# auniquesun/PPT

Measured on AMD Instinct MI355X. Metric: point-clouds/sec fwd+bwd, PointBERT 1024-pt ModelNet40, higher is better.
Workload: dtype f16; 1 GPU; C2: ModelNet40 1024-pt PointBERT (ULIP_PointBERT head_type=0, frozen backbone + PromptLearner), train-mode BN + DropPath, fwd + CE(ls 0.2) + bwd + AdamW; feed=resident, per_gpu_batch=32, global_batch=32, npoints=1024, classes=40, parallelism=dp1

## Files before the change

### include/ppt_hip.h

```cpp
#ifndef PPT_HIP_H
#define PPT_HIP_H

#include <stddef.h>
#include <stdint.h>

#ifdef __cplusplus
extern "C" {
#endif

#define PPT_OK 0
#define PPT_EINVAL (-1)
#define PPT_ELAUNCH (-2)
#define PPT_EUNSUPPORTED (-3)

#define PPT_F32 0
#define PPT_BF16 1
#define PPT_F16 2

const char *ppt_strerror(int code);
int ppt_abi_version(void);

int ppt_fps_f32(const float *xyz, int B, int N, int M, const int64_t *start, int64_t *out_idx,
                float *out_xyz, void *stream);

// ... 210 lines not shown
int ppt_attention_prefix_fwd(const void *qkv, void *out, float *lse, int C, int T, int P, int H, int hd, float scale, int dtype,
                             void *stream);
int ppt_attention_prefix_bwd(const void *qkv, const void *out, const void *dout, const float *lse, float *delta, void *dqkv,
                             float *workspace, int C, int T, int P, int H, int hd, float scale, int dtype, void *stream);

int ppt_conv1_stats(const float *pts, int64_t M, const float *w1, const float *b1, int C,
                    float *part_sum, float *part_sqsum, int *n_partials, void *stream);
int ppt_bn_finalize(const float *part_sum, const float *part_sqsum, int n_partials,
                    int rows_per_partial, int64_t count, int C, const float *gamma, const float *beta, float eps, int train,
                    float momentum, float *running_mean, float *running_var,
                    int64_t *num_batches_tracked, float *scale, float *shift, void *stream);
size_t ppt_bn_finalize_workspace_bytes(int n_partials, int C);
int ppt_bn_finalize_ws(const float *part_sum, const float *part_sqsum, int n_partials,
                       int rows_per_partial, int64_t count, int C, const float *gamma, const float *beta, float eps, int train,
                       float momentum, float *running_mean, float *running_var,
                       int64_t *num_batches_tracked, float *scale, float *shift,
                       float *mean_out , float *rstd_out ,
                       void *workspace, size_t workspace_bytes, void *stream);

int ppt_rows_stats_rows_per_partial(void);
int ppt_rows_stats_f32(const float *x, int64_t M, int C, float *part_sum, float *part_m2, void *stream);
int ppt_bn_rows_bwd_reduce(const float *dy, const float *x, const float *scale, const float *shift, const float *mean,
                           const float *rstd, int relu, int64_t M, int C, float *part_g, float *part_gx, void *stream);
int ppt_bn_rows_bwd_apply(const float *dy, const float *x, const float *scale, const float *shift, const float *mean,
                          const float *rstd, const float *sum_g, const float *sum_gx, int relu, int batch_stats, int64_t M,
                          int C, float *dx, void *dx_half, int half_dtype, void *stream);
int ppt_conv1_stats_max_partials(int64_t M);
int ppt_conv1_stats_rows_per_partial(void);

int ppt_gn_stats_chunks(int R);
int ppt_gn_bwd_chunks(int Q);
int ppt_gn_finish(const double *part, int B, int nch, int G, double n, double eps, int mode, float *out0, float *out1, void *stream);
int ppt_gn_stats(const float *y, int B, int R, int C, int G, double *part, void *stream);
int ppt_gn_lrelu_max(const float *y, const float *mean, const float *rstd, const float *gamma, const float *beta, int B, int Q, int K,
                     int C, int G, float slope, float *out, int32_t *arg, void *stream);
int ppt_gn_bwd_sums(const float *y, const float *dout, const float *out, const int32_t *arg, const float *mean, const float *rstd,
                    const float *gamma, int B, int Q, int K, int C, int G, float slope, double *psum, float *pgb, void *stream);
int ppt_gn_bwd_apply(const float *y, const float *dout, const float *out, const int32_t *arg, const float *mean, const float *rstd,
                     const float *gamma, const float *s12n, int B, int Q, int K, int C, int G, float slope, float *dy, void *stream);

int ppt_mini_pointnet_conv12_bf16(const float *pts, int64_t M, const float *w1, const float *b1, const float *a_scale,
                                  const float *a_shift, int C1, const void *W2, const float *bias2, int N, void *y2, void *gmax,
                                  void *stream);

int ppt_mini_pointnet_conv3_bf16(const void *A, int64_t M, int K, const void *W, const float *gterm, int N, void *y, float *part_sum,
                                 float *part_m2, void *stream);

int ppt_mini_pointnet_conv4_bf16(const void *A, int64_t M, int K, const float *a_scale, const float *a_shift, const void *W,
                                 const float *bias, int N, void *tok, void *stream);

int ppt_mini_pointnet_conv12_half(const float *pts, int64_t M, const float *w1, const float *b1, const float *a_scale,
                                  const float *a_shift, int C1, const void *W2, const float *bias2, int N, void *y2, void *gmax,
                                  int dtype, void *stream);
int ppt_mpn34_retile(const void *W4, void *W4_tiled, void *stream);
int ppt_mini_pointnet_conv34_half(const void *y2, int64_t M, const void *W3s, const float *gs, const void *W4_tiled,
                                  const float *bias4, void *tok, int dtype, void *stream);
int ppt_mini_pointnet_conv3_half(const void *A, int64_t M, int K, const void *W, const float *gterm, int N, void *y, float *part_sum,
                                 float *part_m2, int dtype, void *stream);
int ppt_mini_pointnet_conv4_half(const void *A, int64_t M, int K, const float *a_scale, const float *a_shift, const void *W,
                                 const float *bias, int N, void *tok, int dtype, void *stream);

int ppt_conv12_stats_bf16(const float *pts, int64_t M, const float *w1, const float *b1, const float *a_scale, const float *a_shift,
                          int C1, const void *W2, const float *bias2, int N, void *y2, float *part_sum, float *part_m2, void *stream);

int ppt_affine_conv_pool_bf16(const void *A, int64_t lda, int64_t M, int K, const float *a_scale, const float *a_shift, const void *W,
                              const float *bias, int N, int pool_rows, float *pmax, float *pmin, float *part_sum, float *part_m2,
                              void *stream);

int ppt_group_anchor_stats(const void *x, int x_dtype, const int64_t *idx, const int64_t *anchor, int B, int Nsrc, int S, int K,
                           int D, float *out, void *stream);
int ppt_pointmlp_cloud_rstd(const float *stats, int B, int S, double n, float *r, void *stream);
int ppt_pointmlp_pq(const float *PQ, const float *r, const int64_t *cidx, const float *c0, float *P, float *Q, int B, int N, int S,
                    int C, void *stream);
int ppt_bn_res_act_rows(const void *x, int x_dtype, const void *res, int res_dtype, int64_t M, int C, int pool, const float *scale,
                        const float *shift, const float *res_scale, const float *res_shift, void *y, int y_dtype, void *stream);

int ppt_gemm_tn_bf16(const void *A, int64_t lda, const void *B, int64_t ldb, int64_t M, int N1, int N2, int n_slices, float *part,
                     void *stream);
int ppt_gemm_tn_half(const void *A, int64_t lda, const void *B, int64_t ldb, int64_t M, int N1, int N2, int n_slices, float *part,
                     int dtype, void *stream);

int ppt_cross_entropy_rows(const float *logits, const int64_t *labels, float smoothing, int64_t R, int C, int64_t ignore_index,
                           float *loss, float *dlogits, float *partial, void *stream);

int ppt_rows_matmul_f32(const float *A, const float *W, int M, int K, int N, float alpha, float *out, void *stream);

int ppt_head_logits(const float *feat, const float *w, const float *text, const float *logit_scale, int B, int F, int E, int C,
                    float *spc, float *logits, void *stream);
int ppt_head_ce_bwd(const float *logits, const int64_t *labels, const float *spc, const float *text, float smoothing, int B,
                    int E, int C, float *loss, float *d_text, void *stream);

int ppt_linear3_gelu(const float *pts, int64_t M, const float *w, const float *b, int C, void *y,
                     int y_dtype, void *stream);
int ppt_cls_max_pool(const void *x, int x_dtype, int B, int T, int D, float *out, int32_t *argmax,
                     void *stream);
int ppt_three_nn_interp_fwd(const float *points1, int D1, const float *points2, int D2, const int64_t *idx, const float *dist,
                            int B, int N, int S, void *out, int out_dtype, int ld_out, float *weight_out, void *stream);
int ppt_scatter_rows_bwd(const int64_t *idx, const float *weight, const float *d_rows, int64_t ld, int col_off, int B, int E,
                         int rows_div, int S, int C, float *d_src, void *stream);
int ppt_sum_groups(const float *x, int64_t G, int k, int C, float *out, void *stream);

int ppt_gather_add(const void *P, int p_dtype, const float *Q, const int64_t *idx, int B, int Nsrc, int S, int K,
                   int C, void *y, int y_dtype, float *part_sum, float *part_m2, void *stream);
int ppt_pool_finish(const void *pmax, const void *pmin, int p_dtype, int G, int fold, int C, const float *scale,
                    const float *shift, void *out, int out_dtype, int64_t ld_out, void *stream);
int ppt_bn_act_rows(const float *x, int M, int C, const float *scale, const float *shift, const float *mask,
// ... 72 lines not shown
```

### ppt_amd/_lib.py

```python
import ctypes
import os

_HERE = os.path.dirname(os.path.abspath(__file__))
LIB_PATH = os.environ.get("PPT_HIP_LIB") or os.path.join(_HERE, "csrc", "libppt_hip.so")
_lib = None

PPT_F32, PPT_BF16, PPT_F16 = 0, 1, 2
A_PLAIN, A_AFFINE_RELU, A_CONV1 = 0, 1, 2
ACT_NONE, ACT_RELU, ACT_GELU, ACT_QUICKGELU = 0, 1, 2, 3

c_void_p, c_int, c_int64, c_float, c_size_t = (ctypes.c_void_p, ctypes.c_int, ctypes.c_int64,
                                               ctypes.c_float, ctypes.c_size_t)


class GemmParams(ctypes.Structure):
    _fields_ = [
        ("A", c_void_p), ("lda", c_int64), ("B", c_void_p), ("ldb", c_int64),
        ("C", c_void_p), ("ldc", c_int64), ("M", c_int), ("N", c_int), ("K", c_int),
        ("dtype", c_int), ("c_dtype", c_int),
        ("a_mode", c_int), ("a_scale", c_void_p), ("a_shift", c_void_p), ("pts", c_void_p),
        ("w1", c_void_p), ("b1", c_void_p),
        ("bias", c_void_p), ("group_add", c_void_p), ("group_rows", c_int), ("act", c_int),
        ("dact_pre", c_void_p), ("ld_dact", c_int64),
        ("row_scale", c_void_p), ("row_scale_rows", c_int),
# ... 118 lines not shown
                                  c_void_p, c_int, c_void_p, c_void_p, c_int, c_int, c_int, c_void_p]),
    "ppt_layernorm_fwd_sum": (c_int, [c_void_p, c_void_p, c_void_p, c_int, c_void_p, c_void_p, c_void_p, c_void_p, c_int,
                                      c_void_p, c_void_p, c_int, c_int, c_float, c_void_p]),
    "ppt_layernorm_bwd_sum": (c_int, [c_void_p, c_int, c_void_p, c_void_p, c_void_p, c_void_p, c_void_p, c_int,
                                      c_void_p, c_int, c_int, c_int, c_void_p]),
    "ppt_col_sums": (c_int, [c_void_p, c_int, c_int, c_int, c_int64, c_void_p, c_void_p]),
    "ppt_attention_fwd": (c_int, [c_void_p, c_void_p, c_void_p, c_int, c_int, c_int, c_int, c_float, c_int,
                                  c_int, c_void_p]),
    "ppt_attention_bwd": (c_int, [c_void_p, c_void_p, c_void_p, c_void_p, c_void_p, c_void_p, c_int, c_int,
                                  c_int, c_int, c_float, c_int, c_int, c_void_p]),
    "ppt_attention_prefix_workspace_bytes": (ctypes.c_size_t, [c_int, c_int, c_int, c_int]),
    "ppt_pointmlp_cloud_rstd": (c_int, [c_void_p, c_int, c_int, ctypes.c_double, c_void_p, c_void_p]),
    "ppt_pointmlp_pq": (c_int, [c_void_p, c_void_p, c_void_p, c_void_p, c_void_p, c_void_p, c_int, c_int, c_int, c_int, c_void_p]),
    "ppt_attention_bwd_split16": (c_int, [c_void_p, c_void_p, c_void_p, c_void_p, c_void_p, c_void_p, c_void_p, c_int, c_int, c_int, c_int, c_int, c_float, c_int, c_void_p]),
    "ppt_attention_fwd_split16": (c_int, [c_void_p, c_void_p, c_void_p, c_int, c_int, c_int, c_int, c_int, c_float, c_int, c_void_p]),
    "ppt_attention_prefix_fwd": (c_int, [c_void_p, c_void_p, c_void_p, c_int, c_int, c_int, c_int, c_int, c_float, c_int, c_void_p]),
    "ppt_attention_prefix_bwd": (c_int, [c_void_p, c_void_p, c_void_p, c_void_p, c_void_p, c_void_p, c_void_p, c_int, c_int, c_int,
                                         c_int, c_int, c_float, c_int, c_void_p]),
    "ppt_conv1_stats": (c_int, [c_void_p, c_int64, c_void_p, c_void_p, c_int, c_void_p, c_void_p,
                                ctypes.POINTER(c_int), c_void_p]),
    "ppt_conv1_stats_max_partials": (c_int, [c_int64]),
    "ppt_conv1_stats_rows_per_partial": (c_int, []),
    "ppt_bn_finalize": (c_int, [c_void_p, c_void_p, c_int, c_int, c_int64, c_int, c_void_p, c_void_p, c_float, c_int,
                                c_float, c_void_p, c_void_p, c_void_p, c_void_p, c_void_p, c_void_p]),
    "ppt_bn_finalize_ws": (c_int, [c_void_p, c_void_p, c_int, c_int, c_int64, c_int, c_void_p, c_void_p, c_float, c_int,
                                   c_float, c_void_p, c_void_p, c_void_p, c_void_p, c_void_p, c_void_p, c_void_p, c_void_p,
                                   ctypes.c_size_t, c_void_p]),
    "ppt_rows_stats_rows_per_partial": (c_int, []),
    "ppt_rows_stats_f32": (c_int, [c_void_p, c_int64, c_int, c_void_p, c_void_p, c_void_p]),
    "ppt_bn_rows_bwd_reduce": (c_int, [c_void_p, c_void_p, c_void_p, c_void_p, c_void_p, c_void_p, c_int, c_int64, c_int,
                                       c_void_p, c_void_p, c_void_p]),
    "ppt_bn_rows_bwd_apply": (c_int, [c_void_p, c_void_p, c_void_p, c_void_p, c_void_p, c_void_p, c_void_p, c_void_p, c_int,
                                      c_int, c_int64, c_int, c_void_p, c_void_p, c_int, c_void_p]),
    "ppt_bn_finalize_workspace_bytes": (ctypes.c_size_t, [c_int, c_int]),
    "ppt_gn_stats_chunks": (c_int, [c_int]),
    "ppt_gn_bwd_chunks": (c_int, [c_int]),
    "ppt_gn_stats": (c_int, [c_void_p, c_int, c_int, c_int, c_int, c_void_p, c_void_p]),
    "ppt_gn_lrelu_max": (c_int, [c_void_p, c_void_p, c_void_p, c_void_p, c_void_p, c_int, c_int, c_int, c_int, c_int, c_float,
                                 c_void_p, c_void_p, c_void_p]),
    "ppt_gn_bwd_sums": (c_int, [c_void_p, c_void_p, c_void_p, c_void_p, c_void_p, c_void_p, c_void_p, c_int, c_int, c_int, c_int,
                                c_int, c_float, c_void_p, c_void_p, c_void_p]),
    "ppt_gn_bwd_apply": (c_int, [c_void_p, c_void_p, c_void_p, c_void_p, c_void_p, c_void_p, c_void_p, c_void_p, c_int, c_int,
                                 c_int, c_int, c_int, c_float, c_void_p, c_void_p]),
    "ppt_mini_pointnet_conv12_bf16": (c_int, [c_void_p, c_int64, c_void_p, c_void_p, c_void_p, c_void_p, c_int, c_void_p, c_void_p,
                                              c_int, c_void_p, c_void_p, c_void_p]),
    "ppt_mini_pointnet_conv3_bf16": (c_int, [c_void_p, c_int64, c_int, c_void_p, c_void_p, c_int, c_void_p, c_void_p, c_void_p,
                                             c_void_p]),
    "ppt_mini_pointnet_conv4_bf16": (c_int, [c_void_p, c_int64, c_int, c_void_p, c_void_p, c_void_p, c_void_p, c_int, c_void_p,
                                             c_void_p]),
    "ppt_mini_pointnet_conv12_half": (c_int, [c_void_p, c_int64, c_void_p, c_void_p, c_void_p, c_void_p, c_int, c_void_p, c_void_p,
                                              c_int, c_void_p, c_void_p, c_int, c_void_p]),
    "ppt_mini_pointnet_conv3_half": (c_int, [c_void_p, c_int64, c_int, c_void_p, c_void_p, c_int, c_void_p, c_void_p, c_void_p,
                                             c_int, c_void_p]),
    "ppt_mpn34_retile": (c_int, [c_void_p, c_void_p, c_void_p]),
    "ppt_mini_pointnet_conv34_half": (c_int, [c_void_p, c_int64, c_void_p, c_void_p, c_void_p, c_void_p, c_void_p, c_int, c_void_p]),
    "ppt_mini_pointnet_conv4_half": (c_int, [c_void_p, c_int64, c_int, c_void_p, c_void_p, c_void_p, c_void_p, c_int, c_void_p,
                                             c_int, c_void_p]),
    "ppt_conv12_stats_bf16": (c_int, [c_void_p, c_int64, c_void_p, c_void_p, c_void_p, c_void_p, c_int, c_void_p, c_void_p,
                                      c_int, c_void_p, c_void_p, c_void_p, c_void_p]),
    "ppt_affine_conv_pool_bf16": (c_int, [c_void_p, c_int64, c_int64, c_int, c_void_p, c_void_p, c_void_p, c_void_p, c_int, c_int,
                                          c_void_p, c_void_p, c_void_p, c_void_p, c_void_p]),
    "ppt_group_anchor_stats": (c_int, [c_void_p, c_int, c_void_p, c_void_p, c_int, c_int, c_int, c_int, c_int, c_void_p, c_void_p]),
    "ppt_bn_res_act_rows": (c_int, [c_void_p, c_int, c_void_p, c_int, c_int64, c_int, c_int, c_void_p, c_void_p, c_void_p, c_void_p,
                                    c_void_p, c_int, c_void_p]),
    "ppt_gemm_tn_bf16": (c_int, [c_void_p, c_int64, c_void_p, c_int64, c_int64, c_int, c_int, c_int, c_void_p, c_void_p]),
    "ppt_gemm_tn_half": (c_int, [c_void_p, c_int64, c_void_p, c_int64, c_int64, c_int, c_int, c_int, c_void_p, c_int, c_void_p]),
    "ppt_head_logits": (c_int, [c_void_p, c_void_p, c_void_p, c_void_p, c_int, c_int, c_int, c_int, c_void_p, c_void_p, c_void_p]),
    "ppt_head_ce_bwd": (c_int, [c_void_p, c_void_p, c_void_p, c_void_p, c_float, c_int, c_int, c_int, c_void_p, c_void_p,
                                c_void_p]),
    "ppt_linear3_gelu": (c_int, [c_void_p, c_int64, c_void_p, c_void_p, c_int, c_void_p, c_int, c_void_p]),
    "ppt_cls_max_pool": (c_int, [c_void_p, c_int, c_int, c_int, c_int, c_void_p, c_void_p, c_void_p]),
    "ppt_adamw_step": (c_int, [c_void_p, c_void_p, c_void_p, c_void_p, c_int64, c_float, c_float, c_float, c_float, c_float, c_int,
                               c_float, c_void_p, c_void_p]),
    "ppt_adamw_multi": (c_int, [c_void_p, c_int, c_float, c_float, c_float, c_float, c_float, c_float, c_void_p, c_void_p]),
    "ppt_prompt_rows": (c_int, [c_void_p, c_void_p, c_void_p, c_void_p, c_int, c_int, c_void_p, c_void_p]),
    "ppt_prompt_rows_bwd": (c_int, [c_void_p, c_void_p, c_int, c_int, c_int, c_float, c_void_p, c_void_p]),
    "ppt_convert": (c_int, [c_void_p, c_int, c_void_p, c_int, c_int64, c_void_p]),
    "ppt_weights_prep": (c_int, [c_void_p, c_int, c_int, c_void_p]),
    "ppt_health_check": (c_int, [c_void_p, c_int, c_int64, c_void_p, ctypes.c_uint32, c_void_p, c_void_p]),
    "ppt_labels_check": (c_int, [c_void_p, c_int64, c_int64, c_int64, c_void_p, ctypes.c_uint32, c_void_p]),
    "ppt_scale_rows_convert": (c_int, [c_void_p, c_int64, c_int, c_int, c_void_p, c_void_p, c_int, c_void_p, c_void_p, c_void_p, c_void_p]),
    "ppt_convert_scaled": (c_int, [c_void_p, c_int, c_void_p, c_int, c_int64, c_float, c_void_p]),
    "ppt_transpose": (c_int, [c_void_p, c_int, c_void_p, c_int, c_int, c_int, c_int64, c_void_p]),
    "ppt_reduce_rows": (c_int, [c_void_p, c_int, c_int, c_void_p, c_int, c_void_p]),
    "ppt_cloud_prep_f32": (c_int, [c_void_p, c_int, c_int, c_int, c_void_p, c_void_p, c_int, c_void_p, c_int, c_int, c_int, c_void_p,
                                   c_void_p, c_void_p, c_void_p, c_void_p, c_void_p, c_void_p]),
    "ppt_cloud_draws": (c_int, [c_void_p, c_int, c_void_p, c_int, c_int, ctypes.c_uint64, ctypes.c_uint32, c_void_p, c_void_p,
                                c_void_p, c_void_p, c_void_p, c_void_p, c_int, c_void_p, c_void_p]),
    "ppt_cls_metrics": (c_int, [c_void_p, c_void_p, c_float, c_int, c_int, c_void_p, c_void_p]),
    "ppt_partseg_metrics_chunks": (c_int, [c_int]),
    "ppt_partseg_metrics": (c_int, [c_void_p, c_void_p, c_float, c_int, c_int, c_int, c_void_p, c_void_p, c_int, c_void_p, c_void_p,
                                    c_void_p]),
    "ppt_logreg_workspace_bytes": (ctypes.c_size_t, [c_int, c_int, c_int, c_int]),
    "ppt_logreg_fit_f32": (c_int, [c_void_p, c_int64, c_int, c_void_p, c_void_p, c_int, c_int, c_int, c_int, ctypes.POINTER(c_float),
                                   c_float, c_int, c_void_p, c_void_p, c_void_p, c_void_p, ctypes.c_size_t, c_void_p]),
    "ppt_logreg_predict_f32": (c_int, [c_void_p, c_int64, c_int, c_void_p, c_int, c_void_p, c_void_p, c_int, c_int, c_int, c_void_p,
                                       c_void_p]),
    "ppt_nearest_rows_workspace_bytes": (ctypes.c_size_t, [c_int, c_int, c_int, c_int]),
    "ppt_nearest_rows_f32": (c_int, [c_void_p, c_int, c_void_p, c_int64, c_int, c_int, c_int, c_void_p, c_void_p, c_void_p,
                                     ctypes.c_size_t, c_void_p]),
}


def lib():
    global _lib
    if _lib is None:
# ... 18 lines not shown
```

### ppt_amd/csrc/mpn1.hip

```cpp
#include "group_tile.h"

namespace {

template <typename F, int C1, int TJ, int NWN, bool POOL, bool STATS>
__global__ __launch_bounds__(256) void mpn1_kernel(const float *__restrict__ pts, int n_tiles, const float *__restrict__ w1,
                                                    const float *__restrict__ b1, const float *__restrict__ a_scale,
                                                    const float *__restrict__ a_shift, const bf16_t *__restrict__ W2,
                                                    const float *__restrict__ bias2, bf16_t *__restrict__ y2,
                                                    bf16_t *__restrict__ gmax, float *__restrict__ part_sum,
                                                    float *__restrict__ part_m2)
{
    constexpr int N = 32 * TJ * NWN, KS = C1 / 16, NWM = 4 / NWN;
    constexpr int PITCH = 64 * TJ + 16;
    __shared__ float4 tab[C1];
    __shared__ __align__(16) unsigned char tr_all[4][32 * PITCH];
    const int lane = threadIdx.x & 63;
    const int w = __builtin_amdgcn_readfirstlane(threadIdx.x >> 6);
    const int wn = w % NWN, wm = w / NWN;
    for (int c = threadIdx.x; c < C1; c += 256) {
        const float s = a_scale[c], h = a_shift[c];
        tab[c] = make_float4(s * w1[c * 3 + 0], s * w1[c * 3 + 1], s * w1[c * 3 + 2], fmaf(s, b1[c], h));
    }
    const int col = lane & 31, h = lane >> 5;
    const int n_w = 32 * TJ * wn;
    uint4 bfrag[TJ][KS];
    float bias[TJ];
#pragma unroll
    for (int j = 0; j < TJ; ++j) {
        PPT_GT_LOAD_WEIGHTS(bfrag[j], KS, W2, n_w + 32 * j + col, h);
        bias[j] = bias2 ? bias2[n_w + 32 * j + col] : 0.f;
    }
    unsigned char *tr = tr_all[w];
    __syncthreads();

    for (int t = blockIdx.x * NWM + wm; t < n_tiles; t += gridDim.x * NWM) {
        const float *pp = pts + ((size_t)t * 32 + col) * 3;
        const float x = pp[0], y = pp[1], z = pp[2];
        ppt_f32x16 acc[TJ];
#pragma unroll
        for (int j = 0; j < TJ; ++j)
#pragma unroll
            for (int e = 0; e < 16; ++e) acc[j][e] = 0.f;
#pragma unroll
        for (int s = 0; s < KS; ++s) {
            uint32_t pk[4];
#pragma unroll
            for (int i = 0; i < 4; ++i) {
                const float4 v0 = tab[16 * s + 8 * h + 2 * i], v1 = tab[16 * s + 8 * h + 2 * i + 1];
                const float f0 = fmaxf(fmaf(v0.z, z, fmaf(v0.y, y, fmaf(v0.x, x, v0.w))), 0.0f);
                const float f1 = fmaxf(fmaf(v1.z, z, fmaf(v1.y, y, fmaf(v1.x, x, v1.w))), 0.0f);
                pk[i] = h16<F>::pack2(f0, f1);
            }
            const uint4 a = (make_uint4(pk[0], pk[1], pk[2], pk[3]));
#pragma unroll
            for (int j = 0; j < TJ; ++j) acc[j] = h16<F>::mfma32(a, bfrag[j][s], acc[j]);
        }
#pragma unroll
        for (int j = 0; j < TJ; ++j) {
            float mx = -INFINITY, sm = 0.f;
#pragma unroll
            for (int e = 0; e < 16; ++e) {
                acc[j][e] += bias[j];
                mx = fmaxf(mx, acc[j][e]);
                sm += acc[j][e];
            }
            if constexpr (POOL) {
                mx = xor32_max(mx);
                if (h == 0) gmax[(size_t)t * N + n_w + 32 * j + col] = h16<F>::from_f32(mx);
            }
            if constexpr (STATS) PPT_GT_CHUNK_STATS(acc[j], sm, h, part_sum, part_m2, (size_t)t * N + n_w + 32 * j + col);
            PPT_GT_TILE_TO_LDS(F, acc[j], tr, PITCH, j, lane, col, h);
        }
        PPT_GT_TILE_OUT(TJ, tr, PITCH, y2, (size_t)t * 32, N, n_w, lane);
        __builtin_amdgcn_fence(__ATOMIC_RELEASE, "wavefront");
        __builtin_amdgcn_wave_barrier();
    }
}

int mpn1_grid(int64_t tiles, int nwm, hipStream_t st) { return ppt_persistent_grid((tiles + nwm - 1) / nwm, 3, st); }

}

extern "C" int ppt_mini_pointnet_conv12_half(const float *pts, int64_t M, const float *w1, const float *b1, const float *a_scale,
                                             const float *a_shift, int C1, const void *W2, const float *bias2, int N, void *y2,
                                             void *gmax, int dtype, void *stream)
{
    if (dtype != PPT_BF16 && dtype != PPT_F16) return PPT_EINVAL;
    if (!pts || !w1 || !b1 || !a_scale || !a_shift || !W2 || !bias2 || !y2 || !gmax || M <= 0) return PPT_EINVAL;
    if (C1 != 128 || N != 256 || M % 32) return PPT_EUNSUPPORTED;
    if (((uintptr_t)W2 | (uintptr_t)y2) & 15) return PPT_EINVAL;
    const int64_t tiles = M / 32;
    ppt_launch16(dtype, [&](auto f) {
        hipLaunchKernelGGL((mpn1_kernel<decltype(f), 128, 2, 4, true, false>), dim3(mpn1_grid(tiles, 1, ppt_stream(stream))), dim3(256), 0,
                           ppt_stream(stream), pts, (int)tiles, w1, b1, a_scale, a_shift, (const bf16_t *)W2, bias2, (bf16_t *)y2, (bf16_t *)gmax,
                           nullptr, nullptr);
    });
    PPT_CHECK_LAUNCH();
    return PPT_OK;
}

extern "C" int ppt_mini_pointnet_conv12_bf16(const float *pts, int64_t M, const float *w1, const float *b1, const float *a_scale,
                                             const float *a_shift, int C1, const void *W2, const float *bias2, int N, void *y2,
                                             void *gmax, void *stream)
{
    return ppt_mini_pointnet_conv12_half(pts, M, w1, b1, a_scale, a_shift, C1, W2, bias2, N, y2, gmax, PPT_BF16, stream);
}

extern "C" int ppt_conv12_stats_bf16(const float *pts, int64_t M, const float *w1, const float *b1, const float *a_scale,
                                     const float *a_shift, int C1, const void *W2, const float *bias2, int N, void *y2,
                                     float *part_sum, float *part_m2, void *stream)
{
    if (!pts || !w1 || !b1 || !a_scale || !a_shift || !W2 || !y2 || !part_sum || !part_m2 || M <= 0) return PPT_EINVAL;
    if (M % 32 || (((uintptr_t)W2 | (uintptr_t)y2) & 15)) return PPT_EUNSUPPORTED;
    const int64_t tiles = M / 32;
    hipStream_t s = ppt_stream(stream);
#define MPN_LAUNCH(C, TJ_)                                                                                                 \
    hipLaunchKernelGGL((mpn1_kernel<bf16_t, C, TJ_, 1, false, true>), dim3(mpn1_grid(tiles, 4, s)), dim3(256), 0, s, pts, (int)tiles, w1, b1, \
                       a_scale, a_shift, (const bf16_t *)W2, bias2, (bf16_t *)y2, nullptr, part_sum, part_m2)
    if (C1 == 32 && N == 32) MPN_LAUNCH(32, 1);
    else if (C1 == 64 && N == 64) MPN_LAUNCH(64, 2);
    else if (C1 == 64 && N == 96) MPN_LAUNCH(64, 3);
    else if (C1 == 64 && N == 128) MPN_LAUNCH(64, 4);
    else if (C1 == 128 && N == 128) MPN_LAUNCH(128, 4);
    else return PPT_EUNSUPPORTED;
#undef MPN_LAUNCH
    PPT_CHECK_LAUNCH();
    return PPT_OK;
}
```

### ppt_amd/engine.py

```python
import collections
import os

import torch

from . import ops
from .ops import ACT_GELU, ACT_NONE, ACT_QUICKGELU, A_AFFINE_RELU, A_CONV1

ATTN_SCALE = 64 ** -0.5


class WeightCache:

    def __init__(self, dtype, demoted=None):
        self.dtype = dtype
        self._c = {}
        self.demoted = demoted if demoted is not None else set()

    def get(self, t, kind="w", cols=None, pad_to=None):
        key = (id(t), kind, cols, pad_to)
        ent = self._c.get(key)
        if ent is not None and ent[0] is t and ent[1] == t._version:
            return ent[2]
        with torch.no_grad():
            w = t.detach()
            w = w.reshape(w.shape[0], -1)
            if cols is not None:
                w = w[:, cols[0]:cols[1]].contiguous()
            if pad_to is not None and w.shape[1] % pad_to:
                wp = torch.zeros((w.shape[0], (w.shape[1] + pad_to - 1) // pad_to * pad_to), dtype=w.dtype, device=w.device)
                wp[:, :w.shape[1]] = w
                w = wp
            if kind == "w":
                out = ops.convert(w.contiguous(), self.dtype)
            elif kind == "wt":
                out = ops.transpose(w.contiguous(), self.dtype)
            elif kind == "f32":
                out = w.contiguous()
            else:
                raise ValueError(kind)
        self._c[key] = (t, t._version, out)
        return out

    def derived(self, key, tensors, fn):
        stamp = tuple((id(t), t._version) for t in tensors)
        ent = self._c.get(("derived", key))
        if ent is not None and ent[0] == stamp:
            return ent[2]
        with torch.no_grad():
            out = fn()
        self._c[("derived", key)] = (stamp, tensors, out)
        return out


STAGE_DTYPE = {}


BLOCKS_F16 = os.environ.get("PPT_BLOCKS_F16", "1") != "0"
TOKENIZER_F16 = os.environ.get("PPT_TOKENIZER_F16", "1") != "0"
DECODER_F16 = os.environ.get("PPT_DECODER_F16", "1") != "0"


def _stage_wc(wc, stage):
    dt = STAGE_DTYPE.get(stage)
    if dt is None and wc.dtype == torch.bfloat16 and stage not in wc.demoted:
        if (BLOCKS_F16 and stage in ("blocks", "last_block")) or (TOKENIZER_F16 and stage == "tokenizer"):
            dt = torch.float16
    if dt is None or dt == wc.dtype:
        return wc
    alts = wc.__dict__.setdefault("_alts", {})
    if dt not in alts:
        alts[dt] = WeightCache(dt, wc.demoted)
    return alts[dt]


FUSED_CONV12 = os.environ.get("PPT_FUSED_CONV12", "1") != "0"
FUSED_CONV34 = os.environ.get("PPT_FUSED_CONV34", "1") != "0"
FUSED_CONV34_TRAIN = os.environ.get("PPT_FUSED_CONV34_TRAIN", "0") != "0"
FUSED_MLP = os.environ.get("PPT_FUSED_MLP", "1") != "0"
FUSED_PROJ = os.environ.get("PPT_FUSED_PROJ", "1") != "0"
LNLIN_MAX_ROWS = int(os.environ.get("PPT_LNLIN_MAX_ROWS", "24576"))
BLOCK_PATH = {"qkv": os.environ.get("PPT_BLOCK_QKV", "auto"), "proj": os.environ.get("PPT_BLOCK_PROJ", "fused"),
              "mlp": os.environ.get("PPT_BLOCK_MLP", "fused")}
_RG = os.environ.get("PPT_ROWGEMM", "")
ROWGEMM_MIN_ROWS = 1 << 30 if _RG == "0" else (0 if _RG == "1" else 16000)


def _bn_params(sd, p):
    return (sd[p + "weight"], sd[p + "bias"], sd[p + "running_mean"], sd[p + "running_var"],
            sd[p + "num_batches_tracked"])


def group_points(pc, num_group, group_size, fps_start):
    _, center = ops.fps(pc, num_group, fps_start)
    _, nbhd = ops.knn_group(pc, center, group_size, want_idx=False)
    return nbhd, center


def mini_pointnet(sd, p, wc, nbhd, bn_train, update_running=True):
    B, G, n, _ = nbhd.shape
    assert n == 32, "the fused max-pool epilogue assumes group_size == 32"
    T = wc.dtype
    M = B * G * n
    pts = nbhd.view(M, 3)
    dev = pts.device
    w1 = wc.get(sd[p + "first_conv.0.weight"], "f32")
    b1 = sd[p + "first_conv.0.bias"]
    g1, be1, rm1, rv1, nb1 = _bn_params(sd, p + "first_conv.1.")
    if bn_train:
        ps, pq, rpp = ops.conv1_stats(pts, w1, b1)
        sc1, sh1 = ops.bn_finalize(g1, be1, True, partials=(ps, pq), rows_per_partial=rpp, count=M,
                                   running_mean=rm1, running_var=rv1, num_batches_tracked=nb1,
                                   update_running=update_running)
    else:
        sc1, sh1 = ops.bn_finalize(g1, be1, False, running_mean=rm1, running_var=rv1)
    w2 = wc.get(sd[p + "first_conv.3.weight"])
    if T in ops.HALF and FUSED_CONV12 and tuple(w2.shape) == (256, 128) and w2.stride(0) == 128:
        y2, gmax = ops.mini_pointnet_conv12(pts, w1, b1, sc1, sh1, w2, sd[p + "first_conv.3.bias"])
    else:
        gmax = torch.empty((M // 32, 256), dtype=T, device=dev)
        y2 = ops.gemm(None, w2, out_dtype=T, a_mode=A_CONV1, pts=pts, w1=w1, b1=b1,
                      a_scale=sc1, a_shift=sh1, bias=sd[p + "first_conv.3.bias"], pool_max=gmax)
    w3 = sd[p + "second_conv.0.weight"]
    g2, be2, rm2, rv2, nb2 = _bn_params(sd, p + "second_conv.1.")
    w4p = sd[p + "second_conv.3.weight"]
    fused34 = (FUSED_CONV34 and T in ops.HALF and FUSED_CONV12 and tuple(w3.shape[:2]) == (512, 512) and tuple(w4p.shape[:2]) == (256, 512)
               and y2.is_contiguous() and (not bn_train or FUSED_CONV34_TRAIN))
    if fused34 and not bn_train:
        sc2, sh2 = ops.bn_finalize(g2, be2, False, running_mean=rm2, running_var=rv2)
        w3f = wc.get(w3, "f32")
        w3s_a, b3s = ops.scale_rows_convert(w3f, sc2, T, cols=(0, 256), bias=sd[p + "second_conv.0.bias"], shift=sh2)
        w3s_b = ops.scale_rows_convert(w3f, sc2, T, cols=(256, 512))
        gs = ops.gemm(gmax, w3s_a, out_dtype=torch.float32, bias=b3s, algo_k=0)
        w4t = wc.derived(("mpn34_w4t", p), (w4p,), lambda: ops.mpn34_retile(wc.get(w4p)))
        return ops.mini_pointnet_conv34(y2, w3s_b, gs, w4t, sd[p + "second_conv.3.bias"])
    gterm = ops.gemm(gmax, wc.get(w3, cols=(0, 256)), out_dtype=torch.float32, bias=sd[p + "second_conv.0.bias"],
                     algo_k=0)
    w3b = wc.get(w3, cols=(256, 512))
    fused3 = (T in ops.HALF and FUSED_CONV12 and tuple(w3b.shape) == (512, 256) and w3b.stride(0) == 256
              and y2.is_contiguous() and gterm.is_contiguous())
    if fused34 and fused3:
        cs = torch.empty((M // 32, 512), dtype=torch.float32, device=dev)
        cq = torch.empty_like(cs)
        ops.mini_pointnet_conv3(y2, w3b, gterm, (cs, cq), store=False)
        sc2, sh2 = ops.bn_finalize(g2, be2, True, partials=(cs, cq), rows_per_partial=32, count=M,
                                   running_mean=rm2, running_var=rv2, num_batches_tracked=nb2,
                                   update_running=update_running)
        w3s_b = ops.scale_rows_convert(wc.get(w3, "f32"), sc2, T, cols=(256, 512))
        gs = torch.addcmul(sh2, gterm, sc2)
        w4t = wc.derived(("mpn34_w4t", p), (w4p,), lambda: ops.mpn34_retile(wc.get(w4p)))
        return ops.mini_pointnet_conv34(y2, w3s_b, gs, w4t, sd[p + "second_conv.3.bias"])
    if bn_train:
        cs = torch.empty((M // 32, 512), dtype=torch.float32, device=dev)
        cq = torch.empty_like(cs)
        if fused3:
            y3 = ops.mini_pointnet_conv3(y2, w3b, gterm, (cs, cq))
        else:
            y3 = ops.gemm(y2, w3b, out_dtype=T, group_add=gterm, group_rows=32, col_stats=(cs, cq), algo_k=512)
        sc2, sh2 = ops.bn_finalize(g2, be2, True, partials=(cs, cq), rows_per_partial=32, count=M,
                                   running_mean=rm2, running_var=rv2, num_batches_tracked=nb2,
                                   update_running=update_running)
    else:
        y3 = ops.mini_pointnet_conv3(y2, w3b, gterm) if fused3 else \
            ops.gemm(y2, w3b, out_dtype=T, group_add=gterm, group_rows=32, algo_k=512)
        sc2, sh2 = ops.bn_finalize(g2, be2, False, running_mean=rm2, running_var=rv2)
    w4 = wc.get(sd[p + "second_conv.3.weight"])
    if (T in ops.HALF and FUSED_CONV12 and tuple(w4.shape) == (256, 512) and w4.stride(0) == 512 and y3.is_contiguous()
            and y3.shape[1] == 512):
        return ops.mini_pointnet_conv4(y3, sc2, sh2, w4, sd[p + "second_conv.3.bias"])
    tok = torch.empty((M // 32, w4.shape[0]), dtype=T, device=dev)
    ops.gemm(y3, w4, a_mode=A_AFFINE_RELU, a_scale=sc2, a_shift=sh2, bias=sd[p + "second_conv.3.bias"], pool_max=tok, want_out=False)
    return tok


def _mlp_weights(sd, p, wc):
    w1, w2 = sd[p + "mlp.fc1.weight"], sd[p + "mlp.fc2.weight"]
    return wc.derived(("vit_mlp_tiled", p, ops.VIT_MLP_VARIANT), (w1, w2), lambda: ops.vit_mlp_retile(wc.get(w1), wc.get(w2)))


_VitBlockPlan = collections.namedtuple("_VitBlockPlan", "qkv proj mlp")


def _vit_block_plan(rows, D, hidden, qkv_out, T, keep, pos_in_x, contiguous):
    half = T in ops.HALF
    fusable = FUSED_MLP and half and not keep and D == 384 and hidden == 1536 and contiguous
    if not (rows >= ROWGEMM_MIN_ROWS and half and not keep and D in ops.ROWGEMM_K):
        return _VitBlockPlan("ln_gemm", "fused" if fusable and FUSED_PROJ and rows >= 8192 else "gemm", "fused" if fusable else "gemm")
    qkv, proj, mlp = BLOCK_PATH["qkv"], BLOCK_PATH["proj"], BLOCK_PATH["mlp"]
    if qkv == "auto":
        qkv = "lnlin" if rows <= LNLIN_MAX_ROWS else "rowgemm"
    if qkv not in ("lnlin", "rowgemm"):
        qkv = "ln_gemm"
    elif not pos_in_x:
        qkv = "ln_rowgemm"
    elif qkv == "rowgemm" or qkv_out % 384:
        qkv = "rowgemm_ln"
    mlp = "gemm" if mlp == "v2" else "fused" if mlp == "fused" and fusable else "rowgemm"
    proj = "gemm" if proj == "v2" else "fused" if proj == "fused" and mlp == "fused" and FUSED_PROJ else "rowgemm"
    return _VitBlockPlan(qkv, proj, mlp)


def vit_block_forward(sd, p, wc, x, pos, B, Tn, heads, dp1, dp2, save=None, pos_in_x=False, add_pos_out=False):
    T = wc.dtype
    keep = save is not None
    plan = _vit_block_plan(x.shape[0], x.shape[1], sd[p + "mlp.fc1.weight"].shape[0], sd[p + "attn.qkv.weight"].shape[0], T, keep,
                           pos_in_x, x.is_contiguous())

    def stream():
# ... 744 lines not shown
```

### ppt_amd/ops.py

```python
import ctypes
import os

import torch

from . import _lib
from ._lib import (ACT_GELU, ACT_NONE, ACT_QUICKGELU, ACT_RELU, A_AFFINE_RELU, A_CONV1, A_PLAIN,
                   PPT_BF16, PPT_F16, PPT_F32, GemmParams, RowGemmParams)
from . import _lib as _libmod

_DT = {torch.float32: PPT_F32, torch.bfloat16: PPT_BF16, torch.float16: PPT_F16}
_TORCH_DT = {PPT_F32: torch.float32, PPT_BF16: torch.bfloat16, PPT_F16: torch.float16}
HALF = (torch.bfloat16, torch.float16)


class KernelProfiler:

    def __init__(self):
        self.records = []
        self.kernels = []
        self.executed = []

    def begin(self, name, work, kernel=None, executed=None):
        ev = torch.cuda.Event(enable_timing=True)
        ev.record(torch.cuda.current_stream())
# ... 826 lines not shown
    L = _lib.lib()
    nch = L.ppt_gn_stats_chunks(Q * K)
    part = torch.empty((B, nch, groups, 2), dtype=torch.float64, device=y.device)
    _lib.check(L.ppt_gn_stats(_p(y), B, Q * K, C, groups, _p(part), _stream()), "ppt_gn_stats")
    n = float(Q * K * (C // groups))
    mean = torch.empty((B, groups), dtype=torch.float32, device=y.device)
    rstd = torch.empty((B, groups), dtype=torch.float32, device=y.device)
    _lib.check(L.ppt_gn_finish(_p(part), B, nch, groups, n, float(eps), 0, _p(mean), _p(rstd), _stream()), "ppt_gn_finish")
    out = torch.empty((B, Q, C), dtype=torch.float32, device=y.device)
    arg = torch.empty((B, Q, C), dtype=torch.int32, device=y.device)
    _lib.check(L.ppt_gn_lrelu_max(_p(y), _p(mean), _p(rstd), _p(gamma), _p(beta), B, Q, K, C, groups, slope, _p(out), _p(arg),
                                  _stream()), "ppt_gn_lrelu_max")
    return out, arg, mean, rstd


def gn_lrelu_max_backward(y, dout, out, arg, mean, rstd, gamma, groups, slope):
    _chk(y, torch.float32, "y"); _chk(dout, torch.float32, "dout")
    B, Q, K, C = y.shape
    L = _lib.lib()
    nch = L.ppt_gn_bwd_chunks(Q)
    psum = torch.empty((B, nch, groups, 2), dtype=torch.float64, device=y.device)
    pgb = torch.empty((B, nch, C, 2), dtype=torch.float32, device=y.device)
    _lib.check(L.ppt_gn_bwd_sums(_p(y), _p(dout), _p(out), _p(arg), _p(mean), _p(rstd), _p(gamma), B, Q, K, C, groups, slope,
                                 _p(psum), _p(pgb), _stream()), "ppt_gn_bwd_sums")
    n = float(Q * K * (C // groups))
    s12n = torch.empty((B, groups, 2), dtype=torch.float32, device=y.device)
    _lib.check(L.ppt_gn_finish(_p(psum), B, nch, groups, n, 0.0, 1, _p(s12n), None, _stream()), "ppt_gn_finish")
    gb = reduce_rows(pgb.view(B * nch, 2 * C))
    dy = torch.empty_like(y)
    _lib.check(L.ppt_gn_bwd_apply(_p(y), _p(dout), _p(out), _p(arg), _p(mean), _p(rstd), _p(gamma), _p(s12n), B, Q, K, C, groups,
                                  slope, _p(dy), _stream()), "ppt_gn_bwd_apply")
    gb = gb.view(C, 2)
    return dy, gb[:, 0].contiguous(), gb[:, 1].contiguous()


def mini_pointnet_conv12(pts, w1, b1, a_scale, a_shift, w2, bias2):
    assert w2.dtype in HALF
    _chk(pts, torch.float32, "pts"); _chk(w2, w2.dtype, "w2")
    M = pts.shape[0]
    N, C1 = w2.shape
    y2 = torch.empty((M, N), dtype=w2.dtype, device=pts.device)
    gmax = torch.empty((M // 32, N), dtype=w2.dtype, device=pts.device)
    if profiler is not None:
        profiler.begin("gemm_bf16", 2.0 * M * N * C1, "ppt_mini_pointnet_conv12_bf16")
    _lib.check(_lib.lib().ppt_mini_pointnet_conv12_half(_p(pts), M, _p(w1), _p(b1), _p(a_scale), _p(a_shift), C1, _p(w2), _p(bias2),
                                                        N, _p(y2), _p(gmax), dtype_code(w2), _stream()), "ppt_mini_pointnet_conv12_half")
    if profiler is not None:
        profiler.end()
    if probe is not None:
        _probe("mini-PointNet conv2 output (pre-BN)", y2)
    return y2, gmax


def mini_pointnet_conv3(A, w, gterm, col_stats=None, store=True):
    assert w.dtype in HALF
    _chk(A, w.dtype, "A"); _chk(w, w.dtype, "w"); _chk(gterm, torch.float32, "gterm")
    M, K = A.shape
    N = w.shape[0]
    assert store or col_stats is not None
    y = torch.empty((M, N), dtype=w.dtype, device=A.device) if store else None
    ps, pm = col_stats if col_stats is not None else (None, None)
    if profiler is not None:
        profiler.begin("gemm_bf16", 2.0 * M * N * 2 * K, "ppt_mini_pointnet_conv3_bf16", executed=2.0 * M * N * K)
    _lib.check(_lib.lib().ppt_mini_pointnet_conv3_half(_p(A), M, K, _p(w), _p(gterm), N, _p(y), _p(ps), _p(pm), dtype_code(w), _stream()),
               "ppt_mini_pointnet_conv3_half")
    if profiler is not None:
        profiler.end()
    if probe is not None:
        _probe("mini-PointNet conv3 output (pre-BN)", y)
    return y


def mpn34_retile(w4):
    assert w4.dtype in HALF and tuple(w4.shape) == (256, 512)
    _chk(w4, w4.dtype, "w4")
    out = torch.empty_like(w4)
    _lib.check(_lib.lib().ppt_mpn34_retile(_p(w4), _p(out), _stream()), "ppt_mpn34_retile")
    return out


def mini_pointnet_conv34(y2, w3s, gs, w4_tiled, bias4):
    T = w3s.dtype
    assert T in HALF and tuple(w3s.shape) == (512, 256) and w4_tiled.dtype == T and w4_tiled.numel() == 256 * 512
    _chk(y2, T, "y2"); _chk(w3s, T, "w3s"); _chk(w4_tiled, T, "w4_tiled"); _chk(gs, torch.float32, "gs")
    M = y2.shape[0]
    assert y2.shape[1] == 256 and tuple(gs.shape) == (M // 32, 512) and M % 32 == 0
    tok = torch.empty((M // 32, 256), dtype=T, device=y2.device)
    if profiler is not None:
        profiler.begin("gemm_bf16", 2.0 * M * 512 * 512 + 2.0 * M * 256 * 512, "ppt_mini_pointnet_conv34_half",
                       executed=2.0 * M * 512 * 272 + 2.0 * M * 256 * 512)
    _lib.check(_lib.lib().ppt_mini_pointnet_conv34_half(_p(y2), M, _p(w3s), _p(gs), _p(w4_tiled), _p(bias4), _p(tok), dtype_code(T), _stream()),
               "ppt_mini_pointnet_conv34_half")
    if profiler is not None:
        profiler.end()
    if probe is not None:
        _probe("mini-PointNet tokens", tok)
    return tok


def mini_pointnet_conv4(A, a_scale, a_shift, w, bias):
    assert w.dtype in HALF
    _chk(A, w.dtype, "A"); _chk(w, w.dtype, "w")
    M, K = A.shape
    N = w.shape[0]
    tok = torch.empty((M // 32, N), dtype=w.dtype, device=A.device)
    if profiler is not None:
# ... 426 lines not shown
```

Before: 12460 point-clouds/s.

## Fuse mini-PointNet conv1-conv2-conv3 to avoid materializing conv2 output

Adds a gmax-only pass that computes the conv2 group max without storing the conv2 activation. It also adds a persistent fused kernel that recomputes conv1 and conv2 per tile in LDS and feeds them straight into the conv3 GEMM with column stats. This removes the write and read of the large M×256 y2 tensor in BN-train mode, in exchange for recomputing conv1/conv2 twice and using a heavier LDS footprint and register load.

```diff
diff --git a/include/ppt_hip.h b/include/ppt_hip.h
--- a/include/ppt_hip.h
+++ b/include/ppt_hip.h
@@ -286,6 +286,12 @@
 int ppt_mini_pointnet_conv12_half(const float *pts, int64_t M, const float *w1, const float *b1, const float *a_scale,
                                   const float *a_shift, int C1, const void *W2, const float *bias2, int N, void *y2, void *gmax,
                                   int dtype, void *stream);
+int ppt_mini_pointnet_gmax_half(const float *pts, int64_t M, const float *w1, const float *b1, const float *a_scale,
+                                const float *a_shift, int C1, const void *W2, const float *bias2, int N, void *gmax, int dtype,
+                                void *stream);
+int ppt_mini_pointnet_conv123_half(const float *pts, int64_t M, const float *w1, const float *b1, const float *a_scale,
+                                   const float *a_shift, const void *W2, const float *bias2, const void *W3b, const float *gterm,
+                                   void *y3, float *part_sum, float *part_m2, int dtype, void *stream);
 int ppt_mpn34_retile(const void *W4, void *W4_tiled, void *stream);
 int ppt_mini_pointnet_conv34_half(const void *y2, int64_t M, const void *W3s, const float *gs, const void *W4_tiled,
                                   const float *bias4, void *tok, int dtype, void *stream);
diff --git a/ppt_amd/_lib.py b/ppt_amd/_lib.py
--- a/ppt_amd/_lib.py
+++ b/ppt_amd/_lib.py
@@ -194,6 +194,10 @@
                                               c_int, c_void_p, c_void_p, c_int, c_void_p]),
     "ppt_mini_pointnet_conv3_half": (c_int, [c_void_p, c_int64, c_int, c_void_p, c_void_p, c_int, c_void_p, c_void_p, c_void_p,
                                              c_int, c_void_p]),
+    "ppt_mini_pointnet_gmax_half": (c_int, [c_void_p, c_int64, c_void_p, c_void_p, c_void_p, c_void_p, c_int, c_void_p, c_void_p,
+                                            c_int, c_void_p, c_int, c_void_p]),
+    "ppt_mini_pointnet_conv123_half": (c_int, [c_void_p, c_int64, c_void_p, c_void_p, c_void_p, c_void_p, c_void_p, c_void_p,
+                                               c_void_p, c_void_p, c_void_p, c_void_p, c_void_p, c_int, c_void_p]),
     "ppt_mpn34_retile": (c_int, [c_void_p, c_void_p, c_void_p]),
     "ppt_mini_pointnet_conv34_half": (c_int, [c_void_p, c_int64, c_void_p, c_void_p, c_void_p, c_void_p, c_void_p, c_int, c_void_p]),
     "ppt_mini_pointnet_conv4_half": (c_int, [c_void_p, c_int64, c_int, c_void_p, c_void_p, c_void_p, c_void_p, c_int, c_void_p,
diff --git a/ppt_amd/csrc/mpn1.hip b/ppt_amd/csrc/mpn1.hip
--- a/ppt_amd/csrc/mpn1.hip
+++ b/ppt_amd/csrc/mpn1.hip
@@ -2,7 +2,7 @@
 
 namespace {
 
-template <typename F, int C1, int TJ, int NWN, bool POOL, bool STATS>
+template <typename F, int C1, int TJ, int NWN, bool POOL, bool STATS, bool STORE = true>
 __global__ __launch_bounds__(256) void mpn1_kernel(const float *__restrict__ pts, int n_tiles, const float *__restrict__ w1,
                                                     const float *__restrict__ b1, const float *__restrict__ a_scale,
                                                     const float *__restrict__ a_shift, const bf16_t *__restrict__ W2,
@@ -13,7 +13,7 @@
     constexpr int N = 32 * TJ * NWN, KS = C1 / 16, NWM = 4 / NWN;
     constexpr int PITCH = 64 * TJ + 16;
     __shared__ float4 tab[C1];
-    __shared__ __align__(16) unsigned char tr_all[4][32 * PITCH];
+    __shared__ __align__(16) unsigned char tr_all[STORE ? 4 : 1][STORE ? 32 * PITCH : 16];
     const int lane = threadIdx.x & 63;
     const int w = __builtin_amdgcn_readfirstlane(threadIdx.x >> 6);
     const int wn = w % NWN, wm = w / NWN;
@@ -30,7 +30,7 @@
         PPT_GT_LOAD_WEIGHTS(bfrag[j], KS, W2, n_w + 32 * j + col, h);
         bias[j] = bias2 ? bias2[n_w + 32 * j + col] : 0.f;
     }
-    unsigned char *tr = tr_all[w];
+    unsigned char *tr = tr_all[STORE ? w : 0];
     __syncthreads();
 
     for (int t = blockIdx.x * NWM + wm; t < n_tiles; t += gridDim.x * NWM) {
@@ -69,11 +69,13 @@
                 if (h == 0) gmax[(size_t)t * N + n_w + 32 * j + col] = h16<F>::from_f32(mx);
             }
             if constexpr (STATS) PPT_GT_CHUNK_STATS(acc[j], sm, h, part_sum, part_m2, (size_t)t * N + n_w + 32 * j + col);
-            PPT_GT_TILE_TO_LDS(F, acc[j], tr, PITCH, j, lane, col, h);
+            if constexpr (STORE) PPT_GT_TILE_TO_LDS(F, acc[j], tr, PITCH, j, lane, col, h);
         }
-        PPT_GT_TILE_OUT(TJ, tr, PITCH, y2, (size_t)t * 32, N, n_w, lane);
-        __builtin_amdgcn_fence(__ATOMIC_RELEASE, "wavefront");
-        __builtin_amdgcn_wave_barrier();
+        if constexpr (STORE) {
+            PPT_GT_TILE_OUT(TJ, tr, PITCH, y2, (size_t)t * 32, N, n_w, lane);
+            __builtin_amdgcn_fence(__ATOMIC_RELEASE, "wavefront");
+            __builtin_amdgcn_wave_barrier();
+        }
     }
 }
 
@@ -94,6 +96,24 @@
         hipLaunchKernelGGL((mpn1_kernel<decltype(f), 128, 2, 4, true, false>), dim3(mpn1_grid(tiles, 1, ppt_stream(stream))), dim3(256), 0,
                            ppt_stream(stream), pts, (int)tiles, w1, b1, a_scale, a_shift, (const bf16_t *)W2, bias2, (bf16_t *)y2, (bf16_t *)gmax,
                            nullptr, nullptr);
+    });
+    PPT_CHECK_LAUNCH();
+    return PPT_OK;
+}
+
+extern "C" int ppt_mini_pointnet_gmax_half(const float *pts, int64_t M, const float *w1, const float *b1, const float *a_scale,
+                                           const float *a_shift, int C1, const void *W2, const float *bias2, int N, void *gmax,
+                                           int dtype, void *stream)
+{
+    if (dtype != PPT_BF16 && dtype != PPT_F16) return PPT_EINVAL;
+    if (!pts || !w1 || !b1 || !a_scale || !a_shift || !W2 || !bias2 || !gmax || M <= 0) return PPT_EINVAL;
+    if (C1 != 128 || N != 256 || M % 32) return PPT_EUNSUPPORTED;
+    if ((uintptr_t)W2 & 15) return PPT_EINVAL;
+    const int64_t tiles = M / 32;
+    ppt_launch16(dtype, [&](auto f) {
+        hipLaunchKernelGGL((mpn1_kernel<decltype(f), 128, 4, 2, true, false, false>), dim3(mpn1_grid(tiles, 2, ppt_stream(stream))), dim3(256),
+                           0, ppt_stream(stream), pts, (int)tiles, w1, b1, a_scale, a_shift, (const bf16_t *)W2, bias2, (bf16_t *)nullptr,
+                           (bf16_t *)gmax, nullptr, nullptr);
     });
     PPT_CHECK_LAUNCH();
     return PPT_OK;
diff --git a/ppt_amd/csrc/mpn123.hip b/ppt_amd/csrc/mpn123.hip
--- /dev/null
+++ b/ppt_amd/csrc/mpn123.hip
@@ -0,0 +1,138 @@
+#include "group_lds.h"
+
+namespace {
+
+using G123 = group_lds<256, 2>;
+constexpr int C1_123 = 128, P1_123 = 2 * C1_123 + 16, T1_123 = 32 * P1_123;
+constexpr int LDS_123 = 2 * G123::BUF + 8 * G123::TR + 2 * T1_123 + C1_123 * 16 + 256 * 4;
+
+template <typename F>
+__global__ __launch_bounds__(512, 2) void mpn123_kernel(const float *__restrict__ pts, int n_tiles, const float *__restrict__ w1,
+                                                         const float *__restrict__ b1, const float *__restrict__ a_scale,
+                                                         const float *__restrict__ a_shift, const bf16_t *__restrict__ W2,
+                                                         const float *__restrict__ bias2, const bf16_t *__restrict__ W,
+                                                         const float *__restrict__ add, bf16_t *__restrict__ out,
+                                                         float *__restrict__ part_sum, float *__restrict__ part_m2)
+{
+    using G = G123;
+    constexpr int TJ = G::TJ, KS2 = C1_123 / 16;
+    extern __shared__ __align__(16) unsigned char smem[];
+    const int lane = threadIdx.x & 63;
+    const int w = __builtin_amdgcn_readfirstlane(threadIdx.x >> 6);
+    const int col = lane & 31, h = lane >> 5;
+    const int n_w = 32 * TJ * w;
+    uint4 bfrag[TJ][G::KS];
+#pragma unroll
+    for (int j = 0; j < TJ; ++j) PPT_GT_LOAD_WEIGHTS(bfrag[j], G::KS, W, n_w + 32 * j + col, h);
+    uint4 b2frag[KS2];
+    PPT_GT_LOAD_WEIGHTS(b2frag, KS2, W2, 32 * w + col, h);
+    unsigned char *tr = smem + 2 * G::BUF + w * G::TR;
+    unsigned char *c1 = smem + 2 * G::BUF + 8 * G::TR;
+    float4 *tab = reinterpret_cast<float4 *>(c1 + 2 * T1_123);
+    float *bias_l = reinterpret_cast<float *>(tab + C1_123);
+    if (threadIdx.x >= 256) bias_l[threadIdx.x - 256] = bias2[threadIdx.x - 256];
+    const int cc = threadIdx.x & 15, rb = threadIdx.x >> 4;
+    if (threadIdx.x < C1_123) {
+        const int c = threadIdx.x;
+        const float s = a_scale[c], hh = a_shift[c];
+        tab[16 * (c & 7) + (c >> 3)] = make_float4(s * w1[c * 3 + 0], s * w1[c * 3 + 1], s * w1[c * 3 + 2], fmaf(s, b1[c], hh));
+    }
+    float px, py, pz;
+    auto load = [&](int tile) {
+        const float *pp = pts + ((size_t)tile * 32 + rb) * 3;
+        px = pp[0]; py = pp[1]; pz = pp[2];
+    };
+    auto conv1 = [&](int buf) {
+        uint32_t pk[4];
+#pragma unroll
+        for (int i = 0; i < 4; ++i) {
+            const float4 v0 = tab[16 * (2 * i) + cc], v1 = tab[16 * (2 * i + 1) + cc];
+            const float f0 = fmaxf(fmaf(v0.z, pz, fmaf(v0.y, py, fmaf(v0.x, px, v0.w))), 0.0f);
+            const float f1 = fmaxf(fmaf(v1.z, pz, fmaf(v1.y, py, fmaf(v1.x, px, v1.w))), 0.0f);
+            pk[i] = h16<F>::pack2(f0, f1);
+        }
+        *reinterpret_cast<uint4 *>(c1 + buf * T1_123 + rb * P1_123 + cc * 16) = make_uint4(pk[0], pk[1], pk[2], pk[3]);
+    };
+    auto conv2 = [&](int buf) {
+        const unsigned char *at = c1 + buf * T1_123 + col * P1_123 + 16 * h;
+        ppt_f32x16 acc2;
+#pragma unroll
+        for (int e = 0; e < 16; ++e) acc2[e] = 0.f;
+#pragma unroll
+        for (int s = 0; s < KS2; ++s) acc2 = h16<F>::mfma32(b2frag[s], *reinterpret_cast<const uint4 *>(at + 32 * s), acc2);
+#pragma unroll
+        for (int q = 0; q < 4; ++q) {
+            const float4 bq = *reinterpret_cast<const float4 *>(bias_l + 32 * w + 8 * q + 4 * h);
+            const uint2 pk = make_uint2(h16<F>::pack2(acc2[4 * q] + bq.x, acc2[4 * q + 1] + bq.y),
+                                        h16<F>::pack2(acc2[4 * q + 2] + bq.z, acc2[4 * q + 3] + bq.w));
+            *reinterpret_cast<uint2 *>(smem + buf * G::BUF + col * G::PITCH + 64 * w + 16 * q + 8 * h) = pk;
+        }
+    };
+    int t = blockIdx.x;
+    if (t >= n_tiles) return;
+    const int last = n_tiles - 1, step = (int)gridDim.x;
+    __syncthreads();
+    load(t);
+    conv1(0);
+    load(min(t + step, last));
+    conv1(1);
+    __syncthreads();
+    conv2(0);
+    __syncthreads();
+    for (int it = 0; t < n_tiles; t += step, ++it) {
+        const int cur = it & 1;
+        load(min(t + 2 * step, last));
+        conv2(cur ^ 1);
+        const unsigned char *at = smem + cur * G::BUF + col * G::PITCH + 16 * h;
+        ppt_f32x16 acc[TJ];
+#pragma unroll
+        for (int j = 0; j < TJ; ++j)
+#pragma unroll
+            for (int e = 0; e < 16; ++e) acc[j][e] = 0.f;
+#pragma unroll
+        for (int s = 0; s < G::KS; ++s) {
+            const uint4 a = *reinterpret_cast<const uint4 *>(at + 32 * s);
+#pragma unroll
+            for (int j = 0; j < TJ; ++j) acc[j] = h16<F>::mfma32(a, bfrag[j][s], acc[j]);
+            if (s == 3 || s == 7) __builtin_amdgcn_sched_barrier(0);
+        }
+#pragma unroll
+        for (int j = 0; j < TJ; ++j) {
+            const size_t o = (size_t)t * G::N + n_w + 32 * j + col;
+            const float gt = add[o];
+            float sm = 0.f;
+#pragma unroll
+            for (int e = 0; e < 16; ++e) {
+                acc[j][e] += gt;
+                sm += acc[j][e];
+            }
+            PPT_GT_CHUNK_STATS(acc[j], sm, h, part_sum, part_m2, o);
+            PPT_GT_TILE_TO_LDS(F, acc[j], tr, G::TP, j, lane, col, h);
+        }
+        PPT_GT_TILE_OUT(TJ, tr, G::TP, out, (size_t)t * 32, G::N, n_w, lane);
+        conv1(cur);
+        __syncthreads();
+    }
+}
+
+}
+
+extern "C" int ppt_mini_pointnet_conv123_half(const float *pts, int64_t M, const float *w1, const float *b1, const float *a_scale,
+                                              const float *a_shift, const void *W2, const float *bias2, const void *W3b,
+                                              const float *gterm, void *y3, float *part_sum, float *part_m2, int dtype, void *stream)
+{
+    if (dtype != PPT_BF16 && dtype != PPT_F16) return PPT_EINVAL;
+    if (!pts || !w1 || !b1 || !a_scale || !a_shift || !W2 || !bias2 || !W3b || !gterm || !y3 || !part_sum || !part_m2 || M <= 0)
+        return PPT_EINVAL;
+    if (M % 32) return PPT_EUNSUPPORTED;
+    if (((uintptr_t)W2 | (uintptr_t)W3b | (uintptr_t)y3) & 15) return PPT_EINVAL;
+    PPT_RAISE_LDS_ONCE(LDS_123, (const void *)mpn123_kernel<bf16_t>, (const void *)mpn123_kernel<f16_t>);
+    const int64_t tiles = M / 32;
+    const int grid = ppt_persistent_grid(tiles, 1, ppt_stream(stream));
+    ppt_launch16(dtype, [&](auto f) {
+        hipLaunchKernelGGL(mpn123_kernel<decltype(f)>, dim3(grid), dim3(512), LDS_123, ppt_stream(stream), pts, (int)tiles, w1, b1, a_scale,
+                           a_shift, (const bf16_t *)W2, bias2, (const bf16_t *)W3b, gterm, (bf16_t *)y3, part_sum, part_m2);
+    });
+    PPT_CHECK_LAUNCH();
+    return PPT_OK;
+}
diff --git a/ppt_amd/engine.py b/ppt_amd/engine.py
--- a/ppt_amd/engine.py
+++ b/ppt_amd/engine.py
@@ -76,6 +76,7 @@
 FUSED_CONV12 = os.environ.get("PPT_FUSED_CONV12", "1") != "0"
 FUSED_CONV34 = os.environ.get("PPT_FUSED_CONV34", "1") != "0"
 FUSED_CONV34_TRAIN = os.environ.get("PPT_FUSED_CONV34_TRAIN", "0") != "0"
+FUSED_CONV123 = os.environ.get("PPT_FUSED_CONV123", "1") != "0"
 FUSED_MLP = os.environ.get("PPT_FUSED_MLP", "1") != "0"
 FUSED_PROJ = os.environ.get("PPT_FUSED_PROJ", "1") != "0"
 LNLIN_MAX_ROWS = int(os.environ.get("PPT_LNLIN_MAX_ROWS", "24576"))
@@ -114,17 +115,23 @@
     else:
         sc1, sh1 = ops.bn_finalize(g1, be1, False, running_mean=rm1, running_var=rv1)
     w2 = wc.get(sd[p + "first_conv.3.weight"])
-    if T in ops.HALF and FUSED_CONV12 and tuple(w2.shape) == (256, 128) and w2.stride(0) == 128:
+    w3 = sd[p + "second_conv.0.weight"]
+    fused123 = (FUSED_CONV123 and bn_train and T in ops.HALF and FUSED_CONV12 and ops.probe is None
+                and tuple(w2.shape) == (256, 128) and w2.stride(0) == 128 and tuple(w3.shape[:2]) == (512, 512)
+                and not (FUSED_CONV34 and FUSED_CONV34_TRAIN))
+    if fused123:
+        y2 = None
+        gmax = ops.mini_pointnet_gmax(pts, w1, b1, sc1, sh1, w2, sd[p + "first_conv.3.bias"])
+    elif T in ops.HALF and FUSED_CONV12 and tuple(w2.shape) == (256, 128) and w2.stride(0) == 128:
         y2, gmax = ops.mini_pointnet_conv12(pts, w1, b1, sc1, sh1, w2, sd[p + "first_conv.3.bias"])
     else:
         gmax = torch.empty((M // 32, 256), dtype=T, device=dev)
         y2 = ops.gemm(None, w2, out_dtype=T, a_mode=A_CONV1, pts=pts, w1=w1, b1=b1,
                       a_scale=sc1, a_shift=sh1, bias=sd[p + "first_conv.3.bias"], pool_max=gmax)
-    w3 = sd[p + "second_conv.0.weight"]
     g2, be2, rm2, rv2, nb2 = _bn_params(sd, p + "second_conv.1.")
     w4p = sd[p + "second_conv.3.weight"]
     fused34 = (FUSED_CONV34 and T in ops.HALF and FUSED_CONV12 and tuple(w3.shape[:2]) == (512, 512) and tuple(w4p.shape[:2]) == (256, 512)
-               and y2.is_contiguous() and (not bn_train or FUSED_CONV34_TRAIN))
+               and not fused123 and y2.is_contiguous() and (not bn_train or FUSED_CONV34_TRAIN))
     if fused34 and not bn_train:
         sc2, sh2 = ops.bn_finalize(g2, be2, False, running_mean=rm2, running_var=rv2)
         w3f = wc.get(w3, "f32")
@@ -136,7 +143,7 @@
     gterm = ops.gemm(gmax, wc.get(w3, cols=(0, 256)), out_dtype=torch.float32, bias=sd[p + "second_conv.0.bias"],
                      algo_k=0)
     w3b = wc.get(w3, cols=(256, 512))
-    fused3 = (T in ops.HALF and FUSED_CONV12 and tuple(w3b.shape) == (512, 256) and w3b.stride(0) == 256
+    fused3 = (T in ops.HALF and FUSED_CONV12 and not fused123 and tuple(w3b.shape) == (512, 256) and w3b.stride(0) == 256
               and y2.is_contiguous() and gterm.is_contiguous())
     if fused34 and fused3:
         cs = torch.empty((M // 32, 512), dtype=torch.float32, device=dev)
@@ -152,7 +159,9 @@
     if bn_train:
         cs = torch.empty((M // 32, 512), dtype=torch.float32, device=dev)
         cq = torch.empty_like(cs)
-        if fused3:
+        if fused123:
+            y3 = ops.mini_pointnet_conv123(pts, w1, b1, sc1, sh1, w2, sd[p + "first_conv.3.bias"], w3b, gterm, (cs, cq))
+        elif fused3:
             y3 = ops.mini_pointnet_conv3(y2, w3b, gterm, (cs, cq))
         else:
             y3 = ops.gemm(y2, w3b, out_dtype=T, group_add=gterm, group_rows=32, col_stats=(cs, cq), algo_k=512)
diff --git a/ppt_amd/ops.py b/ppt_amd/ops.py
--- a/ppt_amd/ops.py
+++ b/ppt_amd/ops.py
@@ -902,6 +902,41 @@
     return y2, gmax
 
 
+def mini_pointnet_gmax(pts, w1, b1, a_scale, a_shift, w2, bias2):
+    assert w2.dtype in HALF
+    _chk(pts, torch.float32, "pts"); _chk(w2, w2.dtype, "w2")
+    M = pts.shape[0]
+    N, C1 = w2.shape
+    gmax = torch.empty((M // 32, N), dtype=w2.dtype, device=pts.device)
+    if profiler is not None:
+        profiler.begin("gemm_bf16", 2.0 * M * N * C1, "ppt_mini_pointnet_gmax_half")
+    _lib.check(_lib.lib().ppt_mini_pointnet_gmax_half(_p(pts), M, _p(w1), _p(b1), _p(a_scale), _p(a_shift), C1, _p(w2), _p(bias2),
+                                                      N, _p(gmax), dtype_code(w2), _stream()), "ppt_mini_pointnet_gmax_half")
+    if profiler is not None:
+        profiler.end()
+    return gmax
+
+
+def mini_pointnet_conv123(pts, w1, b1, a_scale, a_shift, w2, bias2, w3b, gterm, col_stats):
+    T = w3b.dtype
+    assert T in HALF and w2.dtype == T and tuple(w2.shape) == (256, 128) and tuple(w3b.shape) == (512, 256)
+    _chk(pts, torch.float32, "pts"); _chk(w2, T, "w2"); _chk(w3b, T, "w3b"); _chk(gterm, torch.float32, "gterm")
+    M = pts.shape[0]
+    ps, pm = col_stats
+    assert M % 32 == 0 and tuple(gterm.shape) == (M // 32, 512) and tuple(ps.shape) == (M // 32, 512) and tuple(pm.shape) == (M // 32, 512)
+    _chk(ps, torch.float32, "part_sum"); _chk(pm, torch.float32, "part_m2")
+    y = torch.empty((M, 512), dtype=T, device=pts.device)
+    if profiler is not None:
+        profiler.begin("gemm_bf16", 2.0 * M * 512 * 512, "ppt_mini_pointnet_conv123_half",
+                       executed=2.0 * M * 512 * 256 + 2.0 * M * 256 * 128)
+    _lib.check(_lib.lib().ppt_mini_pointnet_conv123_half(_p(pts), M, _p(w1), _p(b1), _p(a_scale), _p(a_shift), _p(w2), _p(bias2), _p(w3b),
+                                                         _p(gterm), _p(y), _p(ps), _p(pm), dtype_code(T), _stream()),
+               "ppt_mini_pointnet_conv123_half")
+    if profiler is not None:
+        profiler.end()
+    return y
+
+
 def mini_pointnet_conv3(A, w, gterm, col_stats=None, store=True):
     assert w.dtype in HALF
     _chk(A, w.dtype, "A"); _chk(w, w.dtype, "w"); _chk(gterm, torch.float32, "gterm")
```

Result: no change. 12560 point-clouds/s, median of 6 (+0.8%).
